# graph-embedding/node2vec

Hardware: AMD Instinct MI355X
Metric: walk-steps/sec + embedding-updates/sec on 100M-node synthetic; 1/2/4/8 GPU (higher is better)
Workload: dtype f64

## Files before the change

### node2vec_amd/csrc/n2v_walk_uniform.hip

```cpp
#include "n2v_common.h"

namespace n2v {

__device__ __forceinline__ void rank_row(const n2v_graph &g, const uint32_t *first, const uint32_t *off,
                                         uint32_t x, int64_t &vb, int &n) {
  if (x < (uint32_t)g.rank_head_n) {
    const uint64_t e = g.rank_head[x];
    vb = (int64_t)(e & N2V_HOP_ROW_MASK);
    n = (int)(e >> N2V_HOP_DEG_SHIFT);
    return;
  }
  int c = 0;
  for (int half = g.rank_classes >> 1; half > 0; half >>= 1)
    if (first[c + half] <= x) c += half;
  const uint32_t f0 = first[c], o0 = off[c];
  const uint32_t d = (off[c + 1] - o0) / (first[c + 1] - f0);
  n = (int)d;
  vb = (int64_t)(o0 + (x - f0) * d);
}

constexpr int kChunkMaxL1 = 256;

template <bool kChunked>
struct path_writer;

template <>
struct path_writer<true> {
  int32_t *at;
  int cnt;
  __device__ __forceinline__ path_writer(int32_t *walks_out, int64_t base, int64_t total, int L1, int lane,
                                         int64_t)
      : at(walks_out + base * (int64_t)L1 + lane), cnt((int)(total - base < 64 ? total - base : 64)) {}
  __device__ __forceinline__ void put(int pos, int32_t x, int) { at[pos * cnt] = x; }
};

template <>
struct path_writer<false> {
  int32_t *walks_out;
  int64_t w0;
  int lo;
  bool base_aligned;
  int32_t buf[16];
  __device__ __forceinline__ path_writer(int32_t *out, int64_t, int64_t, int L1, int, int64_t r)
      : walks_out(out), w0(r * (int64_t)L1), lo((int)((r * (int64_t)L1) & 15)),
        base_aligned((reinterpret_cast<uintptr_t>(out) & 63u) == 0) {
#pragma unroll
    for (int k = 0; k < 16; ++k) buf[k] = -1;
  }
  __device__ __forceinline__ void put(int pos, int32_t x, int walk_length) {
    const int64_t a = w0 + pos;
    const int k = (int)(a & 15);
#pragma unroll
    for (int kk = 0; kk < 16; ++kk) buf[kk] = (k == kk) ? x : buf[kk];
    if (k != 15 && pos != walk_length) return;
    int32_t *sec = walks_out + (a & ~(int64_t)15);
    if (lo == 0 && k == 15 && base_aligned) {
#pragma unroll
      for (int u = 0; u < 4; ++u)
        reinterpret_cast<int4 *>(sec)[u] =
            make_int4(buf[4 * u], buf[4 * u + 1], buf[4 * u + 2], buf[4 * u + 3]);
    } else {
#pragma unroll
      for (int kk = 0; kk < 16; ++kk)
        if (kk >= lo && kk <= k) sec[kk] = buf[kk];
    }
    lo = 0;
  }
};

template <int kHops, int kThreads, bool kChunked>
__global__ __launch_bounds__(kThreads, 8) void walk_uniform_kernel(
    n2v_graph g, const int32_t *__restrict__ start_ids, int64_t n_start, int32_t num_walks,
    int32_t walk_length, uint64_t seed, int32_t *__restrict__ walks_out,
    uint8_t *__restrict__ valid_out, uint32_t *__restrict__ status) {
  const int lane = threadIdx.x & 63;
  const int64_t total = n_start * (int64_t)num_walks;
  const int L1 = walk_length + 1;
  extern __shared__ uint32_t rank_lds[];
  const uint32_t *cls_first = rank_lds;
  const uint32_t *cls_where = rank_lds + (kHops >= 3 ? g.rank_classes : 0);
  if (kHops >= 3) {
    for (int c = threadIdx.x; c < g.rank_classes; c += kThreads) {
      rank_lds[c] = g.rank_class_first[c];
      rank_lds[g.rank_classes + c] = g.rank_class_off[c];
    }
    __syncthreads();
  }
  const bool emit_rank = kHops == 3 && g.rank_emit != 0;
  for (;;) {
    uint32_t t = 0;
    if (lane == 0) t = atomicAdd(&status[1], 64u);
    const int64_t base = (int64_t)(uint32_t)__builtin_amdgcn_readfirstlane((int)t);
    if (base >= total) break;
    const int64_t r = base + lane;
    const bool have = r < total;
    int32_t v = -1;
    uint64_t h0 = 0;
    bool alive = have;
    if (have) {
      v = start_ids[r / num_walks];
      const int32_t ordinal = (int32_t)(r % num_walks) + 1;
      h0 = walker_stream(seed, (uint64_t)v * (uint64_t)num_walks + (uint64_t)(ordinal - 1));
      if (v < 0 || (int64_t)v >= g.n_vertices) {
        atomicOr(status, N2V_ST_RANGE);
        alive = false;
      }
    }
    int64_t vb = 0;
    int n = 0;
    int32_t v_emit = v;
    if (kHops >= 3) {
      if (alive) {
        const int32_t rk = g.rank_of[v];
        if (emit_rank) v_emit = rk;
        rank_row(g, cls_first, cls_where, (uint32_t)rk, vb, n);
        alive = n > 0;
      }
    } else if (alive) {
      vb = g.rowptr[v];
      n = (int)(g.rowptr[v + 1] - vb);
      alive = n > 0;
      if (kHops == 2 && g.hop8_rowptr) vb = g.hop8_rowptr[v];
    }
    bool walking = alive;
    auto emit = path_writer<kChunked>(walks_out, base, total, L1, lane, r);
    if (have) emit.put(0, alive ? v_emit : -1, walk_length);
    for (int step = 0; step < walk_length; ++step) {
      if (ballot64(have) == 0ull) break;
      int32_t x = -1;
      if (walking) {
        const uint64_t bits = step_bits(h0, (uint32_t)step);
        const int pick = pick_index((uint32_t)(bits >> 32), n);
        if (kHops == 4) {
          const uint64_t e = reinterpret_cast<const uint64_t *>(g.rank_hops)[vb + pick];
          x = (int32_t)(uint32_t)e;
          if (step + 1 < walk_length) rank_row(g, cls_first, cls_where, (uint32_t)(e >> 32), vb, n);
        } else if (kHops == 3) {
          const uint32_t xr = g.rank_hops[vb + pick];
          x = emit_rank ? (int32_t)xr : g.rank_vertex[xr];
          if (step + 1 < walk_length) rank_row(g, cls_first, cls_where, xr, vb, n);
        } else if (kHops == 2) {
          const uint64_t h = g.hops8[vb + pick];
          const int cb = g.hop8_col_bits, rb = g.hop8_row_bits;
          x = (int32_t)(h & ((1ull << cb) - 1ull));
          vb = (int64_t)(((h >> cb) & ((1ull << rb) - 1ull)) << g.hop8_align_shift);
          const uint64_t code = h >> (cb + rb), esc = (1ull << (64 - cb - rb)) - 1ull;
          n = (int)code;
          if (code == esc) n = (int)(g.rowptr[x + 1] - g.rowptr[x]);
        } else if (kHops == 1) {
          const n2v_hop h = load_hop(g.hops + vb + pick);
          x = h.col;
          vb = hop_row(h);
          n = hop_deg(h);
        } else {
          x = g.col[vb + pick];
          if (step + 1 < walk_length) {
            vb = g.rowptr[x];
            n = (int)(g.rowptr[x + 1] - vb);
          }
        }
        if (step + 1 < walk_length && n == 0) {
          walking = false;
          alive = false;
        }
      }
      if (have) emit.put(step + 1, x, walk_length);
    }
    if (have) valid_out[r] = alive ? 1 : 0;
  }
}

constexpr int kTransposeThreads = 256, kTransposeBatch = 8;

template <int kThreads, int kBatch>
__global__ __launch_bounds__(kThreads) void walk_chunk_transpose_kernel(int32_t *__restrict__ walks,
                                                                        int64_t total, int32_t L1) {
  extern __shared__ int32_t tile[];
  const int m = L1 | 1;
  const int row0 = (int)threadIdx.x / L1, pos0 = (int)threadIdx.x % L1;
  const int drow = kThreads / L1, dpos = kThreads % L1;
  int32_t x[kBatch];
  for (int64_t base = (int64_t)blockIdx.x * 64; base < total; base += (int64_t)gridDim.x * 64) {
    const int cnt = (int)(total - base < 64 ? total - base : 64);
    int32_t *region = walks + base * (int64_t)L1;
    const int n = cnt * L1;
    const bool full = cnt == 64;
    for (int i0 = threadIdx.x; i0 < n; i0 += kThreads * kBatch) {
#pragma unroll
      for (int u = 0; u < kBatch; ++u) {
        const int i = i0 + u * kThreads;
        x[u] = i < n ? region[i] : 0;
      }
#pragma unroll
      for (int u = 0; u < kBatch; ++u) {
        const int i = i0 + u * kThreads;
        const int pos = i >> 6, l = i & 63;
        if (i < n) tile[full ? (pos << 6) + ((l * m + pos) & 63) : i] = x[u];
      }
    }
    __syncthreads();
    int row = row0, pos = pos0;
    for (int i0 = threadIdx.x; i0 < n; i0 += kThreads * kBatch) {
#pragma unroll
      for (int u = 0; u < kBatch; ++u) {
        x[u] = i0 + u * kThreads < n ? tile[pos * cnt + (full ? ((row * m + pos) & 63) : row)] : 0;
        row += drow;
        pos += dpos;
        if (pos >= L1) {
          pos -= L1;
          ++row;
        }
      }
#pragma unroll
      for (int u = 0; u < kBatch; ++u) {
        const int i = i0 + u * kThreads;
        if (i < n) region[i] = x[u];
      }
    }
    __syncthreads();
  }
}

template <int kHops, int kThreads, bool kChunked>
static hipError_t launch_walk_uniform(const n2v_graph *g, const int32_t *start_ids, int64_t n_start,
                                      int32_t num_walks, int32_t walk_length, uint64_t seed, int32_t *walks_out,
                                      uint8_t *valid_out, uint32_t *status, size_t lds, hipStream_t stream) {
  const auto fn = walk_uniform_kernel<kHops, kThreads, kChunked>;
  int64_t blocks = (n_start * (int64_t)num_walks + kThreads - 1) / kThreads;
  const int64_t cap = resident_blocks((const void *)fn, kThreads, lds);
  if (blocks > cap) blocks = cap;
  hipLaunchKernelGGL(fn, dim3((unsigned)blocks), dim3(kThreads), lds, stream, *g, start_ids, n_start, num_walks,
                     walk_length, seed, walks_out, valid_out, status);
  return hipGetLastError();
}

}

extern "C" int n2v_walk_uniform_try(const n2v_graph *g, const int32_t *start_ids, int64_t n_start,
                                    int32_t num_walks, int32_t walk_length, double p, double q,
                                    uint64_t seed, int32_t *walks_out, uint8_t *valid_out,
                                    uint32_t *status, void *stream) {
  if (g->w != nullptr || g->w64 != nullptr || p != 1.0 || q != 1.0) return 0;
  const int64_t total = n_start * (int64_t)num_walks;
  if (total >= 0xffffff00ll) return 0;
  if (total == 0) return 1;
  const int form = g->rank_hops ? (g->rank_emit == 2 ? 4 : 3) : g->hops8 ? 2 : (g->hops ? 1 : 0);
  if (form >= 3) {
    const int P = g->rank_classes;
    if (P < 2 || P > 8192 || (P & (P - 1)) || !g->rank_of || !g->rank_class_first || !g->rank_class_off ||
        g->n_edges >= (1ll << 32) ||
        g->rank_head_n < 0 || g->rank_head_n > (1 << 22) || (g->rank_head_n > 0 && !g->rank_head) ||
        (g->rank_emit == 0 && !g->rank_vertex) || g->rank_emit < 0 || g->rank_emit > 2)
      return N2V_EINVAL;
  }
  if (form == 2 && (g->hop8_col_bits < 1 || g->hop8_row_bits < 1 ||
                    g->hop8_col_bits + g->hop8_row_bits > 62 || g->hop8_align_shift < 0 ||
                    g->hop8_align_shift > 6 || (g->hop8_align_shift > 0 && !g->hop8_rowptr)))
    return N2V_EINVAL;
  if (hipMemsetAsync(status + 1, 0, sizeof(uint32_t), (hipStream_t)stream) != hipSuccess)
    return N2V_ELAUNCH;
  const hipStream_t s = (hipStream_t)stream;
  const size_t lds = form >= 3 ? (size_t)g->rank_classes * 8 : 0;
  const bool chunked = walk_length + 1 <= n2v::kChunkMaxL1;
  hipError_t e = hipSuccess;
#define N2V_UNIFORM_LAUNCH(F, T)                                                                             \
  e = chunked ? n2v::launch_walk_uniform<F, T, true>(g, start_ids, n_start, num_walks, walk_length, seed,    \
                                                     walks_out, valid_out, status, lds, s)                   \
              : n2v::launch_walk_uniform<F, T, false>(g, start_ids, n_start, num_walks, walk_length, seed,   \
                                                      walks_out, valid_out, status, lds, s)
  if (form == 4)
    N2V_UNIFORM_LAUNCH(4, 1024);
  else if (form == 3)
    N2V_UNIFORM_LAUNCH(3, 1024);
  else if (form == 2)
    N2V_UNIFORM_LAUNCH(2, 256);
  else if (form == 1)
    N2V_UNIFORM_LAUNCH(1, 256);
  else
    N2V_UNIFORM_LAUNCH(0, 256);
#undef N2V_UNIFORM_LAUNCH
  if (e != hipSuccess) return N2V_ELAUNCH;
  if (chunked) {
    int64_t chunks = (total + 63) / 64;
    const size_t tile = (size_t)64 * (size_t)(walk_length + 1) * sizeof(int32_t);
    const int64_t cap = n2v::resident_blocks(
        (const void *)n2v::walk_chunk_transpose_kernel<n2v::kTransposeThreads, n2v::kTransposeBatch>,
        n2v::kTransposeThreads, tile);
    if (chunks > cap) chunks = cap;
    hipLaunchKernelGGL((n2v::walk_chunk_transpose_kernel<n2v::kTransposeThreads, n2v::kTransposeBatch>),
                       dim3((unsigned)chunks), dim3(n2v::kTransposeThreads),
                       tile, s, walks_out, total, walk_length + 1);
    if (hipGetLastError() != hipSuccess) return N2V_ELAUNCH;
  }
  return 1;
}
```

Before: 49.14 billion.

## Stage walk output through per-wave LDS ring and drop separate transpose kernel

Replaces the chunked strided writer and its follow-up transpose kernel with a per-wave LDS ring buffer. Each lane deposits its step into LDS, and when lanes complete a 16-word segment the wave cooperatively writes full 64-byte lines to global memory in row-major order. Unaligned head and tail fragments are patched in a finish step. This removes a full extra read and write pass over the walk array and one kernel launch. In exchange it adds LDS usage (about 4.3KB per wave), which may reduce occupancy, plus per-step ballots and wave barriers.

```diff
diff --git a/node2vec_amd/csrc/n2v_walk_uniform.hip b/node2vec_amd/csrc/n2v_walk_uniform.hip
--- a/node2vec_amd/csrc/n2v_walk_uniform.hip
+++ b/node2vec_amd/csrc/n2v_walk_uniform.hip
@@ -19,56 +19,91 @@
   vb = (int64_t)(o0 + (x - f0) * d);
 }
 
-constexpr int kChunkMaxL1 = 256;
-
-template <bool kChunked>
-struct path_writer;
-
-template <>
-struct path_writer<true> {
-  int32_t *at;
-  int cnt;
-  __device__ __forceinline__ path_writer(int32_t *walks_out, int64_t base, int64_t total, int L1, int lane,
-                                         int64_t)
-      : at(walks_out + base * (int64_t)L1 + lane), cnt((int)(total - base < 64 ? total - base : 64)) {}
-  __device__ __forceinline__ void put(int pos, int32_t x, int) { at[pos * cnt] = x; }
+__device__ __forceinline__ void wave_lds_sync() {
+  __builtin_amdgcn_fence(__ATOMIC_RELEASE, "wavefront");
+  __builtin_amdgcn_wave_barrier();
+  __builtin_amdgcn_fence(__ATOMIC_ACQUIRE, "wavefront");
+}
+
+constexpr int kRingPitch = 17;
+constexpr int kRingWords = 64 * kRingPitch;
+
+struct path_writer {
+  int32_t *reg;
+  int32_t *slots;
+  int a0;
+  int first;
+  int L1, cnt, lane;
+  bool ring;
+  int32_t head[15];
+  __device__ __forceinline__ path_writer(int32_t *out, int32_t *wave_slots, int64_t base, int64_t total, int L1_,
+                                         int lane_, int64_t r)
+      : reg(out + base * (int64_t)L1_), slots(wave_slots), a0(0), first(0), L1(L1_),
+        cnt((int)(total - base < 64 ? total - base : 64)), lane(lane_),
+        ring(L1_ >= 32 && L1_ <= (1 << 24) && (reinterpret_cast<uintptr_t>(out) & 63u) == 0) {
+    if (ring) {
+      a0 = lane * L1;
+      first = (a0 + 15) & ~15;
+    } else {
+      reg = out + r * (int64_t)L1_;
+    }
+#pragma unroll
+    for (int k = 0; k < 15; ++k) head[k] = -1;
+  }
+  __device__ __forceinline__ void put(int pos, int32_t x, bool have) {
+    if (!ring) {
+      if (have) reg[pos] = x;
+      return;
+    }
+    const int a = a0 + pos, k = a & 15;
+    if (pos < 15) {
+#pragma unroll
+      for (int kk = 0; kk < 15; ++kk) head[kk] = pos == kk ? x : head[kk];
+    }
+    if (have) slots[lane * kRingPitch + k] = x;
+    const uint64_t done = ballot64(have && k == 15 && a >= first);
+    if (done == 0ull) return;
+    wave_lds_sync();
+    const int q = lane >> 4, w = lane & 15;
+#pragma unroll 1
+    for (uint64_t m = done; m != 0ull;) {
+      int src = -1;
+#pragma unroll
+      for (int u = 0; u < 4; ++u)
+        if (m != 0ull) {
+          const int s = (int)__builtin_ctzll(m);
+          m &= m - 1ull;
+          if (q == u) src = s;
+        }
+      if (src >= 0) reg[((src * L1 + pos) & ~15) + w] = slots[src * kRingPitch + w];
+    }
+    wave_lds_sync();
+  }
+  __device__ __forceinline__ void finish(bool have) {
+    if (!ring || (L1 & 15) == 0) return;
+    wave_lds_sync();
+    int a = a0;
+    asm volatile("" : "+v"(a));
+    const int h = ((a + 15) & ~15) - a;
+    if (have && lane > 0) {
+#pragma unroll
+      for (int kk = 0; kk < 15; ++kk)
+        if (kk < h) slots[(lane - 1) * kRingPitch + ((a + kk) & 15)] = head[kk];
+    }
+    wave_lds_sync();
+    const int q = lane >> 4, w = lane & 15;
+#pragma unroll 1
+    for (int row0 = 0; row0 < cnt; row0 += 4) {
+      const int row = row0 + q;
+      const int end = (row + 1) * L1, t = end & 15;
+      const int nw = row == cnt - 1 ? t : 16;
+      if (row < cnt && t != 0 && w < nw) reg[((end - 1) & ~15) + w] = slots[row * kRingPitch + w];
+    }
+    wave_lds_sync();
+  }
 };
 
-template <>
-struct path_writer<false> {
-  int32_t *walks_out;
-  int64_t w0;
-  int lo;
-  bool base_aligned;
-  int32_t buf[16];
-  __device__ __forceinline__ path_writer(int32_t *out, int64_t, int64_t, int L1, int, int64_t r)
-      : walks_out(out), w0(r * (int64_t)L1), lo((int)((r * (int64_t)L1) & 15)),
-        base_aligned((reinterpret_cast<uintptr_t>(out) & 63u) == 0) {
-#pragma unroll
-    for (int k = 0; k < 16; ++k) buf[k] = -1;
-  }
-  __device__ __forceinline__ void put(int pos, int32_t x, int walk_length) {
-    const int64_t a = w0 + pos;
-    const int k = (int)(a & 15);
-#pragma unroll
-    for (int kk = 0; kk < 16; ++kk) buf[kk] = (k == kk) ? x : buf[kk];
-    if (k != 15 && pos != walk_length) return;
-    int32_t *sec = walks_out + (a & ~(int64_t)15);
-    if (lo == 0 && k == 15 && base_aligned) {
-#pragma unroll
-      for (int u = 0; u < 4; ++u)
-        reinterpret_cast<int4 *>(sec)[u] =
-            make_int4(buf[4 * u], buf[4 * u + 1], buf[4 * u + 2], buf[4 * u + 3]);
-    } else {
-#pragma unroll
-      for (int kk = 0; kk < 16; ++kk)
-        if (kk >= lo && kk <= k) sec[kk] = buf[kk];
-    }
-    lo = 0;
-  }
-};
-
-template <int kHops, int kThreads, bool kChunked>
+template <int kHops, int kThreads>
 __global__ __launch_bounds__(kThreads, 8) void walk_uniform_kernel(
     n2v_graph g, const int32_t *__restrict__ start_ids, int64_t n_start, int32_t num_walks,
     int32_t walk_length, uint64_t seed, int32_t *__restrict__ walks_out,
@@ -87,6 +122,8 @@
     __syncthreads();
   }
   const bool emit_rank = kHops == 3 && g.rank_emit != 0;
+  int32_t *wave_slots = reinterpret_cast<int32_t *>(rank_lds) + (kHops >= 3 ? 2 * g.rank_classes : 0) +
+                        (int)(threadIdx.x >> 6) * kRingWords;
   for (;;) {
     uint32_t t = 0;
     if (lane == 0) t = atomicAdd(&status[1], 64u);
@@ -123,8 +160,8 @@
       if (kHops == 2 && g.hop8_rowptr) vb = g.hop8_rowptr[v];
     }
     bool walking = alive;
-    auto emit = path_writer<kChunked>(walks_out, base, total, L1, lane, r);
-    if (have) emit.put(0, alive ? v_emit : -1, walk_length);
+    auto emit = path_writer(walks_out, wave_slots, base, total, L1, lane, r);
+    emit.put(0, alive ? v_emit : -1, have);
     for (int step = 0; step < walk_length; ++step) {
       if (ballot64(have) == 0ull) break;
       int32_t x = -1;
@@ -164,68 +201,22 @@
           alive = false;
         }
       }
-      if (have) emit.put(step + 1, x, walk_length);
-    }
+      emit.put(step + 1, x, have);
+    }
+    emit.finish(have);
     if (have) valid_out[r] = alive ? 1 : 0;
   }
 }
 
-constexpr int kTransposeThreads = 256, kTransposeBatch = 8;
-
-template <int kThreads, int kBatch>
-__global__ __launch_bounds__(kThreads) void walk_chunk_transpose_kernel(int32_t *__restrict__ walks,
-                                                                        int64_t total, int32_t L1) {
-  extern __shared__ int32_t tile[];
-  const int m = L1 | 1;
-  const int row0 = (int)threadIdx.x / L1, pos0 = (int)threadIdx.x % L1;
-  const int drow = kThreads / L1, dpos = kThreads % L1;
-  int32_t x[kBatch];
-  for (int64_t base = (int64_t)blockIdx.x * 64; base < total; base += (int64_t)gridDim.x * 64) {
-    const int cnt = (int)(total - base < 64 ? total - base : 64);
-    int32_t *region = walks + base * (int64_t)L1;
-    const int n = cnt * L1;
-    const bool full = cnt == 64;
-    for (int i0 = threadIdx.x; i0 < n; i0 += kThreads * kBatch) {
-#pragma unroll
-      for (int u = 0; u < kBatch; ++u) {
-        const int i = i0 + u * kThreads;
-        x[u] = i < n ? region[i] : 0;
-      }
-#pragma unroll
-      for (int u = 0; u < kBatch; ++u) {
-        const int i = i0 + u * kThreads;
-        const int pos = i >> 6, l = i & 63;
-        if (i < n) tile[full ? (pos << 6) + ((l * m + pos) & 63) : i] = x[u];
-      }
-    }
-    __syncthreads();
-    int row = row0, pos = pos0;
-    for (int i0 = threadIdx.x; i0 < n; i0 += kThreads * kBatch) {
-#pragma unroll
-      for (int u = 0; u < kBatch; ++u) {
-        x[u] = i0 + u * kThreads < n ? tile[pos * cnt + (full ? ((row * m + pos) & 63) : row)] : 0;
-        row += drow;
-        pos += dpos;
-        if (pos >= L1) {
-          pos -= L1;
-          ++row;
-        }
-      }
-#pragma unroll
-      for (int u = 0; u < kBatch; ++u) {
-        const int i = i0 + u * kThreads;
-        if (i < n) region[i] = x[u];
-      }
-    }
-    __syncthreads();
-  }
-}
-
-template <int kHops, int kThreads, bool kChunked>
+template <int kHops, int kThreads>
 static hipError_t launch_walk_uniform(const n2v_graph *g, const int32_t *start_ids, int64_t n_start,
                                       int32_t num_walks, int32_t walk_length, uint64_t seed, int32_t *walks_out,
                                       uint8_t *valid_out, uint32_t *status, size_t lds, hipStream_t stream) {
-  const auto fn = walk_uniform_kernel<kHops, kThreads, kChunked>;
+  const auto fn = walk_uniform_kernel<kHops, kThreads>;
+  lds += (size_t)(kThreads / 64) * kRingWords * sizeof(int32_t);
+  if (lds > 64 * 1024 && hipFuncSetAttribute((const void *)fn, hipFuncAttributeMaxDynamicSharedMemorySize,
+                                             (int)lds) != hipSuccess)
+    return hipErrorInvalidValue;
   int64_t blocks = (n_start * (int64_t)num_walks + kThreads - 1) / kThreads;
   const int64_t cap = resident_blocks((const void *)fn, kThreads, lds);
   if (blocks > cap) blocks = cap;
@@ -261,13 +252,10 @@
     return N2V_ELAUNCH;
   const hipStream_t s = (hipStream_t)stream;
   const size_t lds = form >= 3 ? (size_t)g->rank_classes * 8 : 0;
-  const bool chunked = walk_length + 1 <= n2v::kChunkMaxL1;
   hipError_t e = hipSuccess;
-#define N2V_UNIFORM_LAUNCH(F, T)                                                                             \
-  e = chunked ? n2v::launch_walk_uniform<F, T, true>(g, start_ids, n_start, num_walks, walk_length, seed,    \
-                                                     walks_out, valid_out, status, lds, s)                   \
-              : n2v::launch_walk_uniform<F, T, false>(g, start_ids, n_start, num_walks, walk_length, seed,   \
-                                                      walks_out, valid_out, status, lds, s)
+#define N2V_UNIFORM_LAUNCH(F, T)                                                                         \
+  e = n2v::launch_walk_uniform<F, T>(g, start_ids, n_start, num_walks, walk_length, seed, walks_out, valid_out, \
+                                     status, lds, s)
   if (form == 4)
     N2V_UNIFORM_LAUNCH(4, 1024);
   else if (form == 3)
@@ -280,17 +268,5 @@
     N2V_UNIFORM_LAUNCH(0, 256);
 #undef N2V_UNIFORM_LAUNCH
   if (e != hipSuccess) return N2V_ELAUNCH;
-  if (chunked) {
-    int64_t chunks = (total + 63) / 64;
-    const size_t tile = (size_t)64 * (size_t)(walk_length + 1) * sizeof(int32_t);
-    const int64_t cap = n2v::resident_blocks(
-        (const void *)n2v::walk_chunk_transpose_kernel<n2v::kTransposeThreads, n2v::kTransposeBatch>,
-        n2v::kTransposeThreads, tile);
-    if (chunks > cap) chunks = cap;
-    hipLaunchKernelGGL((n2v::walk_chunk_transpose_kernel<n2v::kTransposeThreads, n2v::kTransposeBatch>),
-                       dim3((unsigned)chunks), dim3(n2v::kTransposeThreads),
-                       tile, s, walks_out, total, walk_length + 1);
-    if (hipGetLastError() != hipSuccess) return N2V_ELAUNCH;
-  }
   return 1;
 }
```

New measurement: 50.99 billion, median of 3. 1.04x the previous value.
